# imatge-upc/rsis

Hardware: AMD Instinct MI355X
Metric: training images/sec at 256x256, T=10, batch=32 per GPU (higher is better)
Workload: dtype f32

## Files before the change

### rsis_amd/csrc/conv_wgrad_tiled.hip

```cpp
#include "common.h"
#include <stdlib.h>

typedef __attribute__((address_space(3))) void* lds_vp_t;

struct WgradTiledArgs {
  const float* dy;
  const float* x;
  float* dw;
  int B, Cs, H, W, Cout;
  int ldo, n_off, interleave_hid;
  int n_co_tiles, n_n_tiles, n_sp_tiles, tiles_per_split;
};

#define RSIS_OOB 0x7FFFFFF0u

template <int BM, int BN, int WGM, int WGN, int KS, int TW, int KSP = 1, int RAG = 0>
__device__ __forceinline__ void wgrad_tiled_body(const WgradTiledArgs& p, const int bx, const int by) {
#if __HIP_DEVICE_COMPILE__
  constexpr int TM = BM / WGM / 32, TN = BN / WGN / 32;
  constexpr int KK = KS * KS, HALO = KS / 2;
  constexpr int TP = KS == 1 ? 32 : 64;
  constexpr int TH = TP / TW;
  constexpr int NG = TP / 4;
  constexpr int GPR = TW / 4;
  constexpr int PW = TW + 2 * HALO, PH = TH + 2 * HALO, IMS = PW * PH;
  constexpr int CI_P = KS == 1 ? BN : (BN + KK - 2) / KK + 1;
  constexpr int AS = BM * TP;
  constexpr int XS = KS == 1 ? BN * TP : (CI_P * IMS + 255) / 256 * 256;
  constexpr int NA = BM * NG / 256;
  constexpr int NB4 = KS == 1 ? BN * NG / 256 : 0;
  constexpr int NB1 = KS == 1 ? 0 : XS / 256;
  static_assert(WGM * WGN * KSP == 4 && (BM * NG) % 256 == 0 && (KS == 3 || (BN * NG) % 256 == 0) && (NG / 2) % KSP == 0, "config");

  __shared__ __attribute__((aligned(16))) float lds[2 * (AS + XS)];
  float* const As0 = lds;
  float* const Xs0 = lds + 2 * AS;

  const int tid = threadIdx.x, lane = tid & 63, l31 = lane & 31, hi = lane >> 5;
  const int wave = __builtin_amdgcn_readfirstlane(tid >> 6);
  const int wk = wave / (WGM * WGN), wm = (wave % (WGM * WGN)) / WGN, wn = wave % WGN;
  const int H = p.H, W = p.W, HW = H * W, Cs = p.Cs, Cout = p.Cout;
  const int co_t = bx % p.n_co_tiles, n_t = bx / p.n_co_tiles;
  const int co0 = co_t * BM, n0 = n_t * BN;
  const int ci0 = n0 / KK;
  const int Nn = Cs * KK;
  const int tiles_x = RAG ? (W + TW - 1) / TW : W / TW, tiles_y = RAG ? (H + TH - 1) / TH : H / TH;
  const int rx = W - (tiles_x - 1) * TW, ry = H - (tiles_y - 1) * TH;
  const int t_begin = by * p.tiles_per_split;
  const int t_end = min(t_begin + p.tiles_per_split, p.n_sp_tiles);
  if (t_begin >= t_end) return;

  unsigned voa[NA];
#pragma unroll
  for (int i = 0; i < NA; ++i) {
    const int idx = tid + i * 256;
    const int row = idx / NG, sl = idx % NG;
    const int G = (sl & ~7) | ((sl & 7) ^ (row & 7));
    const int y = G / GPR, x4 = G % GPR;
    voa[i] = co0 + row < Cout ? ((unsigned)((co0 + row) * HW + y * W + x4 * 4) * 4u) | (RAG == 2 && x4 * 4 >= rx ? 1u : 0u) | (RAG == 2 && y >= ry ? 2u : 0u) : RSIS_OOB;
  }
  unsigned voa1[RAG == 1 ? 4 * NA : 1];
  unsigned vob1r[RAG == 1 && NB4 ? 4 * NB4 : 1];
  if constexpr (RAG == 1) {
#pragma unroll
    for (int k = 0; k < 4 * NA; ++k) {
      const int P = k * 256 + tid, idx = P >> 2, e = P & 3;
      const int row = idx / NG, sl = idx % NG;
      const int G = (sl & ~7) | ((sl & 7) ^ (row & 7));
      const int y = G / GPR, x = (G % GPR) * 4 + e;
      voa1[k] = co0 + row < Cout ? ((unsigned)((co0 + row) * HW + y * W + x) * 4u) | (x >= rx ? 1u : 0u) | (y >= ry ? 2u : 0u) : RSIS_OOB;
    }
    if constexpr (KS == 1) {
#pragma unroll
      for (int k = 0; k < 4 * NB4; ++k) {
        const int P = k * 256 + tid, idx = P >> 2, e = P & 3;
        const int row = idx / NG, sl = idx % NG;
        const int G = (sl & ~7) | ((sl & 7) ^ (row & 7));
        const int y = G / GPR, x = (G % GPR) * 4 + e;
        vob1r[k] = n0 + row < Cs ? ((unsigned)((n0 + row) * HW + y * W + x) * 4u) | (x >= rx ? 1u : 0u) | (y >= ry ? 2u : 0u) : RSIS_OOB;
      }
    }
  }
  unsigned vob4[NB4 ? NB4 : 1];
  unsigned vob1[NB1 ? NB1 : 1];
  unsigned cls1[NB1 ? NB1 : 1];
  if constexpr (KS == 1) {
#pragma unroll
    for (int i = 0; i < NB4; ++i) {
      const int idx = tid + i * 256;
      const int row = idx / NG, sl = idx % NG;
      const int G = (sl & ~7) | ((sl & 7) ^ (row & 7));
      const int y = G / GPR, x4 = G % GPR;
      vob4[i] = n0 + row < Cs ? ((unsigned)((n0 + row) * HW + y * W + x4 * 4) * 4u) | (RAG == 2 && x4 * 4 >= rx ? 1u : 0u) | (RAG == 2 && y >= ry ? 2u : 0u) : RSIS_OOB;
    }
  } else {
#pragma unroll
    for (int i = 0; i < NB1; ++i) {
      const int e = tid + i * 256;
      const int cl = e / IMS, rem = e - cl * IMS;
      const int py = rem / PW, pxx = rem - py * PW;
      const bool ok = cl < CI_P && ci0 + cl < Cs;
      vob1[i] = ok ? (unsigned)(cl * HW + py * W + pxx) * 4u : RSIS_OOB;
      cls1[i] = (py == 0 ? 1u : 0u) | (py - 1 >= ry ? 2u : 0u) | (pxx == 0 ? 4u : 0u) | (pxx - 1 >= rx ? 8u : 0u);
    }
  }

  int sg[NG / 2 / KSP];
  int bo[NG / 2 / KSP];
#pragma unroll
  for (int gg = 0; gg < NG / 2 / KSP; ++gg) {
    const int g = gg * KSP + (KSP == 1 ? 0 : wk);
    sg[gg] = ((2 * g + hi) ^ (l31 & 7)) * 4;
    bo[gg] = KS == 1 ? 0 : (g / (TW / 8)) * PW + (g % (TW / 8)) * 8;
  }
  const int arow = (wm * TM * 32 + l31) * TP;
  int xb[TN];
#pragma unroll
  for (int j = 0; j < TN; ++j) {
    const int nl = wn * TN * 32 + j * 32 + l31;
    if constexpr (KS == 1) {
      xb[j] = nl * TP;
    } else {
      const int n = n0 + nl;
      const int cl = n / KK - ci0, rs = n - (n / KK) * KK;
      xb[j] = cl * IMS + (rs / KS) * PW + (rs % KS) + 4 * hi;
    }
  }

  f32x16 acc[TM][TN];
#pragma unroll
  for (int i = 0; i < TM; ++i)
#pragma unroll
    for (int j = 0; j < TN; ++j)
#pragma unroll
      for (int r = 0; r < 16; ++r) acc[i][j][r] = 0.f;

  int tb = t_begin / (tiles_x * tiles_y);
  int trem = t_begin - tb * (tiles_x * tiles_y);
  int ty = trem / tiles_x, tx = trem - ty * tiles_x;

#define WG_ISSUE(BUF)                                                                                          \
  {                                                                                                            \
    const int y0 = ty * TH, x0 = tx * TW;                                                                      \
    const float* ab = p.dy + ((size_t)tb * Cout * HW + y0 * W + x0);                                           \
    const __amdgpu_buffer_rsrc_t ra_ = __builtin_amdgcn_make_buffer_rsrc((void*)ab, 0, 0x7FFFFFF0, 0x00020000); \
    const unsigned lastm = (tx == tiles_x - 1 ? 1u : 0u) | (ty == tiles_y - 1 ? 2u : 0u);                      \
    if constexpr (RAG == 1) {                                                                                  \
      float* As = As0 + (BUF) * AS + wave * 64;                                                                \
      _Pragma("unroll") for (int k = 0; k < 4 * NA; ++k)                                                       \
        __builtin_amdgcn_raw_ptr_buffer_load_lds(ra_, (lds_vp_t)(As + k * 256), 4, (voa1[k] & lastm) ? RSIS_OOB : (voa1[k] & ~3u), 0, 0, 0); \
    } else {                                                                                                   \
      float* As = As0 + (BUF) * AS + wave * 256;                                                               \
      _Pragma("unroll") for (int i = 0; i < NA; ++i)                                                           \
        __builtin_amdgcn_raw_ptr_buffer_load_lds(ra_, (lds_vp_t)(As + i * 1024), 16,                           \
                                                 RAG == 2 ? ((voa[i] & lastm) ? RSIS_OOB : (voa[i] & ~3u)) : voa[i], 0, 0, 0); \
    }                                                                                                          \
    if constexpr (KS == 1) {                                                                                   \
      const float* bb = p.x + ((size_t)tb * Cs * HW + y0 * W + x0);                                            \
      const __amdgpu_buffer_rsrc_t rb_ = __builtin_amdgcn_make_buffer_rsrc((void*)bb, 0, 0x7FFFFFF0, 0x00020000); \
      if constexpr (RAG == 1) {                                                                                \
        float* Xs = Xs0 + (BUF) * XS + wave * 64;                                                              \
        _Pragma("unroll") for (int k = 0; k < 4 * NB4; ++k)                                                    \
          __builtin_amdgcn_raw_ptr_buffer_load_lds(rb_, (lds_vp_t)(Xs + k * 256), 4, (vob1r[k] & lastm) ? RSIS_OOB : (vob1r[k] & ~3u), 0, 0, 0); \
      } else {                                                                                                 \
        float* Xs = Xs0 + (BUF) * XS + wave * 256;                                                             \
        _Pragma("unroll") for (int i = 0; i < NB4; ++i)                                                        \
          __builtin_amdgcn_raw_ptr_buffer_load_lds(rb_, (lds_vp_t)(Xs + i * 1024), 16,                         \
                                                   RAG == 2 ? ((vob4[i] & lastm) ? RSIS_OOB : (vob4[i] & ~3u)) : vob4[i], 0, 0, 0); \
      }                                                                                                        \
    } else {                                                                                                   \
      const float* bb = p.x + (((size_t)tb * Cs + ci0) * HW + (y0 - 1) * W + (x0 - 1));                        \
      const __amdgpu_buffer_rsrc_t rb_ = __builtin_amdgcn_make_buffer_rsrc((void*)bb, 0, 0x7FFFFFF0, 0x00020000); \
      const unsigned edge = (y0 == 0 ? 1u : 0u) | (ty == tiles_y - 1 ? 2u : 0u) | (x0 == 0 ? 4u : 0u) | (tx == tiles_x - 1 ? 8u : 0u); \
      float* Xs = Xs0 + (BUF) * XS + wave * 64;                                                                \
      _Pragma("unroll") for (int i = 0; i < NB1; ++i) {                                                        \
        const unsigned vo = (cls1[i] & edge) ? RSIS_OOB : vob1[i];                                             \
        __builtin_amdgcn_raw_ptr_buffer_load_lds(rb_, (lds_vp_t)(Xs + i * 256), 4, vo, 0, 0, 0);               \
      }                                                                                                        \
    }                                                                                                          \
    if (++tx == tiles_x) { tx = 0; if (++ty == tiles_y) { ty = 0; ++tb; } }                                    \
  }
#define WG_LAND() __builtin_amdgcn_s_waitcnt(0x0F70);

  WG_ISSUE(0)
  WG_LAND()
  __syncthreads();
  const int ntl = t_end - t_begin;
  for (int t = 0; t < ntl; ++t) {
    const int cur = t & 1;
    if (t + 1 < ntl) WG_ISSUE(cur ^ 1)
    {
      const float* As = As0 + cur * AS + arow;
      const float* Xs = Xs0 + cur * XS;
#pragma unroll
      for (int g = 0; g < NG / 2 / KSP; ++g) {
        f32x4 a4[TM];
#pragma unroll
        for (int i = 0; i < TM; ++i) a4[i] = *reinterpret_cast<const f32x4*>(As + i * 32 * TP + sg[g]);
        if constexpr (KS == 1) {
          f32x4 b4[TN];
#pragma unroll
          for (int j = 0; j < TN; ++j) b4[j] = *reinterpret_cast<const f32x4*>(Xs + xb[j] + sg[g]);
#pragma unroll
          for (int e = 0; e < 4; ++e)
#pragma unroll
            for (int i = 0; i < TM; ++i)
#pragma unroll
              for (int j = 0; j < TN; ++j) acc[i][j] = __builtin_amdgcn_mfma_f32_32x32x2f32(a4[i][e], b4[j][e], acc[i][j], 0, 0, 0);
        } else {
#pragma unroll
          for (int e = 0; e < 4; ++e) {
            float b[TN];
#pragma unroll
            for (int j = 0; j < TN; ++j) b[j] = Xs[xb[j] + (KSP == 1 ? (g / (TW / 8)) * PW + (g % (TW / 8)) * 8 : bo[g]) + e];
#pragma unroll
            for (int i = 0; i < TM; ++i)
#pragma unroll
              for (int j = 0; j < TN; ++j) acc[i][j] = __builtin_amdgcn_mfma_f32_32x32x2f32(a4[i][e], b[j], acc[i][j], 0, 0, 0);
          }
        }
      }
    }
    WG_LAND()
    __syncthreads();
  }
#undef WG_ISSUE
#undef WG_LAND

  const __amdgpu_buffer_rsrc_t rdw = __builtin_amdgcn_make_buffer_rsrc((void*)p.dw, 0, (unsigned)((size_t)Cout * p.ldo * 4), 0x00020000);
  const int ihid = p.interleave_hid;
  const unsigned ldb = (unsigned)p.ldo * 4u;
#pragma unroll
  for (int j = 0; j < TN; ++j) {
    const int n = n0 + wn * TN * 32 + j * 32 + l31;
    if (n >= Nn) continue;
#pragma unroll
    for (int i = 0; i < TM; ++i) {
      const int row0 = co0 + wm * TM * 32 + i * 32 + 4 * hi;
      const int rows_left = Cout - row0;
      const unsigned vo = (unsigned)((ihid > 0 ? row0 >> 2 : row0) * p.ldo + p.n_off + n) * 4u;
#pragma unroll
      for (int r = 0; r < 16; ++r) {
        const int k = (r & 3) + 8 * (r >> 2);
        const unsigned ro = (unsigned)(ihid > 0 ? (r & 3) * ihid + 2 * (r >> 2) : k) * ldb;
        __builtin_amdgcn_raw_ptr_buffer_atomic_fadd_f32(acc[i][j][r], rdw, k < rows_left ? vo + ro : 0x7FFFFFF0u, 0, 0);
      }
    }
  }
#endif
}

template <int BM, int BN, int WGM, int WGN, int KS, int TW, int KSP = 1>
__global__ __launch_bounds__(256) void conv_wgrad_tiled_kernel(const WgradTiledArgs p) {
  wgrad_tiled_body<BM, BN, WGM, WGN, KS, TW, KSP>(p, blockIdx.x, blockIdx.y);
}

#define RSIS_WG_MAXJ 48
struct WgradTiledGroup {
  int n;
  int begin[RSIS_WG_MAXJ + 1];
  WgradTiledArgs job[RSIS_WG_MAXJ];
};
static_assert(sizeof(WgradTiledGroup) <= 4000, "kernel arguments are limited to 4 KB");

template <int BM, int BN, int WGM, int WGN, int KS, int TW, int KSP = 1, int RAG = 0>
__global__ __launch_bounds__(256) void conv_wgrad_tiled_group_kernel(const WgradTiledGroup g) {
  const int b = blockIdx.x;
  int lo = 0, hi = g.n - 1;
  while (lo < hi) {
    const int mid = (lo + hi + 1) >> 1;
    if (g.begin[mid] <= b) lo = mid; else hi = mid - 1;
  }
  const WgradTiledArgs& p = g.job[lo];
  const int local = b - g.begin[lo];
  const int ntile = p.n_co_tiles * p.n_n_tiles;
  wgrad_tiled_body<BM, BN, WGM, WGN, KS, TW, KSP, RAG>(p, local % ntile, local / ntile);
}

template <int BM, int BN, int WGM, int WGN, int KS, int TW, int KSP = 1>
static int launch_tiled_cfg(WgradTiledArgs& a, hipStream_t st) {
  constexpr int TH = (KS == 1 ? 32 : 64) / TW;
  a.n_co_tiles = rsis_cdiv(a.Cout, BM);
  a.n_n_tiles = rsis_cdiv((long)a.Cs * KS * KS, BN);
  a.n_sp_tiles = a.B * (a.H / TH) * (a.W / TW);
  const int ntile = a.n_co_tiles * a.n_n_tiles;
  const int slots = KS == 1 ? (BM * BN >= 128 * 128 ? 256 : 512) : 256 * (BM * BN >= 128 * 128 ? 2 : 3);
  int nsplit = ntile >= slots ? 1 : slots / ntile;
  if (nsplit > a.n_sp_tiles / 2) nsplit = a.n_sp_tiles / 2;
  if (nsplit < 1 || rsis_deterministic()) nsplit = 1;
  a.tiles_per_split = rsis_cdiv(a.n_sp_tiles, nsplit);
  nsplit = rsis_cdiv(a.n_sp_tiles, a.tiles_per_split);
  hipLaunchKernelGGL((conv_wgrad_tiled_kernel<BM, BN, WGM, WGN, KS, TW, KSP>), dim3(ntile, nsplit), dim3(256), 0, st, a);
  return rsis_check_launch();
}

template <int KS, int TW>
static int launch_tiled_tw(WgradTiledArgs& a, hipStream_t st) {
  const int nmod = (a.Cs * KS * KS) % 128;
  const bool narrow = nmod != 0 && nmod <= 64;
  if (rsis_deterministic() && a.Cout <= 32) return launch_tiled_cfg<32, 128, 1, 4, KS, TW>(a, st);
  if (KS == 1 && a.Cout > 32) return launch_tiled_cfg<64, 64, 2, 2, KS, TW>(a, st);
  if (a.Cout <= 32) return narrow ? launch_tiled_cfg<32, 64, 1, 2, KS, TW, 2>(a, st) : launch_tiled_cfg<32, 128, 1, 4, KS, TW>(a, st);
  if (a.Cout <= 64) return narrow ? launch_tiled_cfg<64, 64, 2, 2, KS, TW>(a, st) : launch_tiled_cfg<64, 128, 2, 2, KS, TW>(a, st);
  return narrow ? launch_tiled_cfg<128, 64, 2, 2, KS, TW>(a, st) : launch_tiled_cfg<128, 128, 2, 2, KS, TW>(a, st);
}

static int tiled_tw(int H, int W, int ks) {
  const int tp = ks == 1 ? 32 : 64;
  for (int tw = ks == 1 ? 32 : 16; tw >= 8; tw >>= 1)
    if (W % tw == 0 && H % (tp / tw) == 0) return tw;
  return 0;
}
static int tiled_tw_ragged(int W, int ks) {
  const int wide = ks == 1 ? 32 : 16;
  return W > 16 ? wide : (W > 8 ? 16 : 8);
}

static int tiled_cfg_code(const WgradTiledArgs& a, int ks) {
  const int nmod = (a.Cs * ks * ks) % 128;
  const bool narrow = nmod != 0 && nmod <= 64;
  if (ks == 1 && a.Cout > 32) return 2;
  if (a.Cout <= 32) return narrow && !rsis_deterministic() ? 0 : 1;
  if (a.Cout <= 64) return narrow ? 2 : 3;
  return narrow ? 4 : 5;
}

template <int BM, int BN, int WGM, int WGN, int KS, int TW, int KSP = 1, int RAG = 0>
static int launch_group_cfg(WgradTiledArgs* jobs, int n, hipStream_t st) {
  constexpr int TH = (KS == 1 ? 32 : 64) / TW;
  long total_iters = 0;
  for (int j = 0; j < n; ++j) {
    WgradTiledArgs& a = jobs[j];
    a.n_co_tiles = rsis_cdiv(a.Cout, BM);
    a.n_n_tiles = rsis_cdiv((long)a.Cs * KS * KS, BN);
    a.n_sp_tiles = RAG ? a.B * rsis_cdiv(a.H, TH) * rsis_cdiv(a.W, TW) : a.B * (a.H / TH) * (a.W / TW);
    total_iters += (long)a.n_co_tiles * a.n_n_tiles * a.n_sp_tiles;
  }
  static const int env_tb = getenv("RSIS_WG_GROUP_BLOCKS") ? atoi(getenv("RSIS_WG_GROUP_BLOCKS")) : 0;
  const long target_blocks = env_tb > 0 ? env_tb : 2048;
  long L = (total_iters + target_blocks - 1) / target_blocks;
  if (L < 2) L = 2;
  if (rsis_deterministic()) L = 1L << 40;
  for (int j0 = 0; j0 < n; j0 += RSIS_WG_MAXJ) {
    WgradTiledGroup g;
    g.n = n - j0 < RSIS_WG_MAXJ ? n - j0 : RSIS_WG_MAXJ;
    int blocks = 0;
    for (int j = 0; j < g.n; ++j) {
      WgradTiledArgs a = jobs[j0 + j];
      int nsplit = rsis_cdiv(a.n_sp_tiles, L);
      if (nsplit < 1) nsplit = 1;
      a.tiles_per_split = rsis_cdiv(a.n_sp_tiles, nsplit);
      nsplit = rsis_cdiv(a.n_sp_tiles, a.tiles_per_split);
      g.begin[j] = blocks;
      g.job[j] = a;
      blocks += a.n_co_tiles * a.n_n_tiles * nsplit;
    }
    g.begin[g.n] = blocks;
    hipLaunchKernelGGL((conv_wgrad_tiled_group_kernel<BM, BN, WGM, WGN, KS, TW, KSP, RAG>), dim3(blocks), dim3(256), 0, st, g);
    if (rsis_check_launch() != RSIS_OK) return RSIS_ERR_LAUNCH;
  }
  return RSIS_OK;
}

template <int KS, int TW, int RAG = 0>
static int launch_group_tw(int code, WgradTiledArgs* jobs, int n, hipStream_t st) {
  switch (code) {
    case 0: return launch_group_cfg<32, 64, 1, 2, KS, TW, 2, RAG>(jobs, n, st);
    case 1: return launch_group_cfg<32, 128, 1, 4, KS, TW, 1, RAG>(jobs, n, st);
    case 2: return launch_group_cfg<64, 64, 2, 2, KS, TW, 1, RAG>(jobs, n, st);
    case 3: return launch_group_cfg<64, 128, 2, 2, KS, TW, 1, RAG>(jobs, n, st);
    case 4: return launch_group_cfg<128, 64, 2, 2, KS, TW, 1, RAG>(jobs, n, st);
    default: return launch_group_cfg<128, 128, 2, 2, KS, TW, 1, RAG>(jobs, n, st);
  }
}

int rsis_launch_conv_wgrad_tiled_group(const WgradArgs* w, int n, int ks, hipStream_t st) {
  if (n < 1) return RSIS_OK;
  WgradTiledArgs* all = (WgradTiledArgs*)malloc(sizeof(WgradTiledArgs) * n * 2);
  int* key = (int*)malloc(sizeof(int) * n);
  if (!all || !key) { free(all); free(key); return RSIS_ERR_LAUNCH; }
  WgradTiledArgs* bucket = all + n;
  for (int j = 0; j < n; ++j) {
    WgradTiledArgs a = {};
    a.dy = w[j].dy; a.x = w[j].x; a.dw = w[j].dw; a.B = w[j].B; a.Cs = w[j].Cs; a.H = w[j].H; a.W = w[j].W; a.Cout = w[j].Cout;
    a.ldo = w[j].ldo; a.n_off = w[j].n_off; a.interleave_hid = w[j].interleave_hid;
    all[j] = a;
    const int twa = tiled_tw(a.H, a.W, ks);
    if (twa) key[j] = twa * 8 + tiled_cfg_code(a, ks);
    else {
      if (ks == 1 && (a.H * a.W) % 4 == 0) { all[j].W = a.W = a.H * a.W; all[j].H = a.H = 1; }
      key[j] = (a.W % 4 == 0 ? 2048 : 1024) + tiled_tw_ragged(a.W, ks) * 8 + tiled_cfg_code(a, ks);
    }
  }
  int rc = RSIS_OK;
  for (int j = 0; j < n && rc == RSIS_OK; ++j) {
    if (key[j] < 0) continue;
    const int k = key[j];
    int m = 0;
    for (int i = j; i < n; ++i)
      if (key[i] == k) { bucket[m++] = all[i]; key[i] = -1; }
    const int rag = k >> 10;
    const int tw = (k & 1023) / 8, code = k % 8;
    if (rag == 1) {
      if (ks == 1) rc = tw == 32 ? launch_group_tw<1, 32, 1>(code, bucket, m, st) : (tw == 16 ? launch_group_tw<1, 16, 1>(code, bucket, m, st) : launch_group_tw<1, 8, 1>(code, bucket, m, st));
      else rc = tw == 16 ? launch_group_tw<3, 16, 1>(code, bucket, m, st) : launch_group_tw<3, 8, 1>(code, bucket, m, st);
    } else if (rag == 2) {
      if (ks == 1) rc = tw == 32 ? launch_group_tw<1, 32, 2>(code, bucket, m, st) : (tw == 16 ? launch_group_tw<1, 16, 2>(code, bucket, m, st) : launch_group_tw<1, 8, 2>(code, bucket, m, st));
      else rc = tw == 16 ? launch_group_tw<3, 16, 2>(code, bucket, m, st) : launch_group_tw<3, 8, 2>(code, bucket, m, st);
    } else if (ks == 1) rc = tw == 32 ? launch_group_tw<1, 32>(code, bucket, m, st) : (tw == 16 ? launch_group_tw<1, 16>(code, bucket, m, st) : launch_group_tw<1, 8>(code, bucket, m, st));
    else rc = tw == 16 ? launch_group_tw<3, 16>(code, bucket, m, st) : launch_group_tw<3, 8>(code, bucket, m, st);
  }
  free(all); free(key);
  return rc;
}

bool rsis_wgrad_tiled_supported(const WgradArgs& w, int ks) {
  if (!(ks == 1 || ks == 3) || w.stride != 1 || w.pad != ks / 2 || w.H != w.Ho || w.W != w.Wo) return false;
  static const bool ragged_on = !(getenv("RSIS_WGRAD_RAGGED") && getenv("RSIS_WGRAD_RAGGED")[0] == '0');
  if (tiled_tw(w.H, w.W, ks) == 0 && !ragged_on) return false;
  const long img = (long)w.H * w.W * 4;
  return (long)w.Cout * img < (1L << 30) && (long)w.Cs * img < (1L << 30);
}

int rsis_launch_conv_wgrad_tiled(const WgradArgs& w, int ks, hipStream_t st) {
  WgradTiledArgs a = {};
  a.dy = w.dy; a.x = w.x; a.dw = w.dw; a.B = w.B; a.Cs = w.Cs; a.H = w.H; a.W = w.W; a.Cout = w.Cout;
  a.ldo = w.ldo; a.n_off = w.n_off; a.interleave_hid = w.interleave_hid;
  const int tw = tiled_tw(w.H, w.W, ks);
  if (tw == 0) return rsis_launch_conv_wgrad_tiled_group(&w, 1, ks, st);
  if (ks == 1) {
    if (tw == 32) return launch_tiled_tw<1, 32>(a, st);
    if (tw == 16) return launch_tiled_tw<1, 16>(a, st);
    return launch_tiled_tw<1, 8>(a, st);
  }
  if (tw == 16) return launch_tiled_tw<3, 16>(a, st);
  return launch_tiled_tw<3, 8>(a, st);
}
```

Before: 905.7.

## Emulate fp32 wgrad MFMA with three-limb bf16 split products

Adds a limb path to the tiled weight-gradient kernel. Each fp32 operand is split into three truncated bf16 limbs, and six cross products are accumulated with 32x32x16 bf16 MFMA in place of the fp32 32x32x2 MFMA. The path is enabled by default only for selected kernel-size, tile-width and config codes, and an environment variable can override it. The aim is to use the much higher bf16 matrix throughput while keeping accuracy close to fp32, at the cost of extra split and pack ALU work per LDS load and slightly lower precision from dropping the low-order limb products.

```diff
diff --git a/rsis_amd/csrc/conv_wgrad_tiled.hip b/rsis_amd/csrc/conv_wgrad_tiled.hip
--- a/rsis_amd/csrc/conv_wgrad_tiled.hip
+++ b/rsis_amd/csrc/conv_wgrad_tiled.hip
@@ -1,7 +1,30 @@
 #include "common.h"
+#include "limb_split.h"
 #include <stdlib.h>
+#include <string.h>
 
 typedef __attribute__((address_space(3))) void* lds_vp_t;
+typedef __bf16 wg_bf16x8 __attribute__((ext_vector_type(8)));
+typedef unsigned wg_u32x4 __attribute__((ext_vector_type(4)));
+
+#define WG_LIMB_PRODUCTS 6
+[[maybe_unused]] __device__ constexpr int wg_limb_pa[9] = {2, 1, 0, 1, 0, 0, 2, 1, 2};
+[[maybe_unused]] __device__ constexpr int wg_limb_pb[9] = {0, 1, 2, 0, 1, 0, 1, 2, 2};
+
+__device__ __forceinline__ void wg_limb_pack8(const float (&v)[8], wg_bf16x8 (&out)[3]) {
+  wg_u32x4 q[3];
+#pragma unroll
+  for (int m = 0; m < 4; ++m) {
+    float lo[3], hi[3];
+    rsis_limb_split3(v[2 * m], lo[0], lo[1], lo[2]);
+    rsis_limb_split3(v[2 * m + 1], hi[0], hi[1], hi[2]);
+    q[0][m] = __builtin_amdgcn_perm(__float_as_uint(v[2 * m + 1]), __float_as_uint(v[2 * m]), 0x07060302u);
+    q[1][m] = __builtin_amdgcn_perm(__float_as_uint(hi[1]), __float_as_uint(lo[1]), 0x07060302u);
+    q[2][m] = __builtin_amdgcn_perm(__float_as_uint(hi[2]), __float_as_uint(lo[2]), 0x07060302u);
+  }
+#pragma unroll
+  for (int l = 0; l < 3; ++l) out[l] = __builtin_bit_cast(wg_bf16x8, q[l]);
+}
 
 struct WgradTiledArgs {
   const float* dy;
@@ -14,7 +37,7 @@
 
 #define RSIS_OOB 0x7FFFFFF0u
 
-template <int BM, int BN, int WGM, int WGN, int KS, int TW, int KSP = 1, int RAG = 0>
+template <int BM, int BN, int WGM, int WGN, int KS, int TW, int KSP = 1, int RAG = 0, int LIMB = 0>
 __device__ __forceinline__ void wgrad_tiled_body(const WgradTiledArgs& p, const int bx, const int by) {
 #if __HIP_DEVICE_COMPILE__
   constexpr int TM = BM / WGM / 32, TN = BN / WGN / 32;
@@ -30,7 +53,7 @@
   constexpr int NA = BM * NG / 256;
   constexpr int NB4 = KS == 1 ? BN * NG / 256 : 0;
   constexpr int NB1 = KS == 1 ? 0 : XS / 256;
-  static_assert(WGM * WGN * KSP == 4 && (BM * NG) % 256 == 0 && (KS == 3 || (BN * NG) % 256 == 0) && (NG / 2) % KSP == 0, "config");
+  static_assert(WGM * WGN * KSP == 4 && (BM * NG) % 256 == 0 && (KS == 3 || (BN * NG) % 256 == 0) && (NG / 2) % KSP == 0 && (NG / 2 / KSP) % 2 == 0, "config");
 
   __shared__ __attribute__((aligned(16))) float lds[2 * (AS + XS)];
   float* const As0 = lds;
@@ -192,6 +215,43 @@
     {
       const float* As = As0 + cur * AS + arow;
       const float* Xs = Xs0 + cur * XS;
+      if constexpr (LIMB) {
+#pragma unroll
+        for (int g = 0; g < NG / 2 / KSP; g += 2) {
+          wg_bf16x8 al[TM][3], bl[TN][3];
+#pragma unroll
+          for (int i = 0; i < TM; ++i) {
+            const f32x4 a0 = *reinterpret_cast<const f32x4*>(As + i * 32 * TP + sg[g]);
+            const f32x4 a1 = *reinterpret_cast<const f32x4*>(As + i * 32 * TP + sg[g + 1]);
+            const float v[8] = {a0[0], a0[1], a0[2], a0[3], a1[0], a1[1], a1[2], a1[3]};
+            wg_limb_pack8(v, al[i]);
+          }
+#pragma unroll
+          for (int j = 0; j < TN; ++j) {
+            float v[8];
+            if constexpr (KS == 1) {
+              const f32x4 b0 = *reinterpret_cast<const f32x4*>(Xs + xb[j] + sg[g]);
+              const f32x4 b1 = *reinterpret_cast<const f32x4*>(Xs + xb[j] + sg[g + 1]);
+#pragma unroll
+              for (int e = 0; e < 4; ++e) { v[e] = b0[e]; v[4 + e] = b1[e]; }
+            } else {
+#pragma unroll
+              for (int u = 0; u < 2; ++u)
+#pragma unroll
+                for (int e = 0; e < 4; ++e)
+                  v[4 * u + e] = Xs[xb[j] + (KSP == 1 ? ((g + u) / (TW / 8)) * PW + ((g + u) % (TW / 8)) * 8 : bo[g + u]) + e];
+            }
+            wg_limb_pack8(v, bl[j]);
+          }
+#pragma unroll
+          for (int q = 0; q < WG_LIMB_PRODUCTS; ++q)
+#pragma unroll
+            for (int i = 0; i < TM; ++i)
+#pragma unroll
+              for (int j = 0; j < TN; ++j)
+                acc[i][j] = __builtin_amdgcn_mfma_f32_32x32x16_bf16(al[i][wg_limb_pa[q]], bl[j][wg_limb_pb[q]], acc[i][j], 0, 0, 0);
+        }
+      } else
 #pragma unroll
       for (int g = 0; g < NG / 2 / KSP; ++g) {
         f32x4 a4[TM];
@@ -250,9 +310,9 @@
 #endif
 }
 
-template <int BM, int BN, int WGM, int WGN, int KS, int TW, int KSP = 1>
+template <int BM, int BN, int WGM, int WGN, int KS, int TW, int KSP = 1, int LIMB = 0>
 __global__ __launch_bounds__(256) void conv_wgrad_tiled_kernel(const WgradTiledArgs p) {
-  wgrad_tiled_body<BM, BN, WGM, WGN, KS, TW, KSP>(p, blockIdx.x, blockIdx.y);
+  wgrad_tiled_body<BM, BN, WGM, WGN, KS, TW, KSP, 0, LIMB>(p, blockIdx.x, blockIdx.y);
 }
 
 #define RSIS_WG_MAXJ 48
@@ -263,7 +323,7 @@
 };
 static_assert(sizeof(WgradTiledGroup) <= 4000, "kernel arguments are limited to 4 KB");
 
-template <int BM, int BN, int WGM, int WGN, int KS, int TW, int KSP = 1, int RAG = 0>
+template <int BM, int BN, int WGM, int WGN, int KS, int TW, int KSP = 1, int RAG = 0, int LIMB = 0>
 __global__ __launch_bounds__(256) void conv_wgrad_tiled_group_kernel(const WgradTiledGroup g) {
   const int b = blockIdx.x;
   int lo = 0, hi = g.n - 1;
@@ -274,10 +334,25 @@
   const WgradTiledArgs& p = g.job[lo];
   const int local = b - g.begin[lo];
   const int ntile = p.n_co_tiles * p.n_n_tiles;
-  wgrad_tiled_body<BM, BN, WGM, WGN, KS, TW, KSP, RAG>(p, local % ntile, local / ntile);
-}
-
-template <int BM, int BN, int WGM, int WGN, int KS, int TW, int KSP = 1>
+  wgrad_tiled_body<BM, BN, WGM, WGN, KS, TW, KSP, RAG, LIMB>(p, local % ntile, local / ntile);
+}
+
+static unsigned wg_limb_mask(int ks, int tw) {
+  if (ks == 3) return tw == 16 ? 0x3Fu : (tw == 8 ? 1u << 5 : 0u);
+  return tw == 16 || tw == 8 ? 1u << 2 : 0u;
+}
+static bool wg_use_limbs(int ks, int tw, int code, int rag) {
+  static const int mode = [] {
+    const char* e = getenv("RSIS_WGRAD_LIMBS");
+    if (!e || !e[0]) return 0;
+    if (e[0] == '0') return 1;
+    return strcmp(e, "all") == 0 ? 2 : 0;
+  }();
+  if (mode) return mode == 2;
+  return rag == 0 && ((wg_limb_mask(ks, tw) >> code) & 1u);
+}
+
+template <int BM, int BN, int WGM, int WGN, int KS, int TW, int KSP = 1, int LIMB = 0>
 static int launch_tiled_cfg(WgradTiledArgs& a, hipStream_t st) {
   constexpr int TH = (KS == 1 ? 32 : 64) / TW;
   a.n_co_tiles = rsis_cdiv(a.Cout, BM);
@@ -290,19 +365,28 @@
   if (nsplit < 1 || rsis_deterministic()) nsplit = 1;
   a.tiles_per_split = rsis_cdiv(a.n_sp_tiles, nsplit);
   nsplit = rsis_cdiv(a.n_sp_tiles, a.tiles_per_split);
-  hipLaunchKernelGGL((conv_wgrad_tiled_kernel<BM, BN, WGM, WGN, KS, TW, KSP>), dim3(ntile, nsplit), dim3(256), 0, st, a);
+  hipLaunchKernelGGL((conv_wgrad_tiled_kernel<BM, BN, WGM, WGN, KS, TW, KSP, LIMB>), dim3(ntile, nsplit), dim3(256), 0, st, a);
   return rsis_check_launch();
 }
+
+template <int KS, int TW, int LIMB>
+static int launch_tiled_code(int code, WgradTiledArgs& a, hipStream_t st) {
+  switch (code) {
+    case 0: return launch_tiled_cfg<32, 64, 1, 2, KS, TW, 2, LIMB>(a, st);
+    case 1: return launch_tiled_cfg<32, 128, 1, 4, KS, TW, 1, LIMB>(a, st);
+    case 2: return launch_tiled_cfg<64, 64, 2, 2, KS, TW, 1, LIMB>(a, st);
+    case 3: return launch_tiled_cfg<64, 128, 2, 2, KS, TW, 1, LIMB>(a, st);
+    case 4: return launch_tiled_cfg<128, 64, 2, 2, KS, TW, 1, LIMB>(a, st);
+    default: return launch_tiled_cfg<128, 128, 2, 2, KS, TW, 1, LIMB>(a, st);
+  }
+}
+
+static int tiled_cfg_code(const WgradTiledArgs& a, int ks);
 
 template <int KS, int TW>
 static int launch_tiled_tw(WgradTiledArgs& a, hipStream_t st) {
-  const int nmod = (a.Cs * KS * KS) % 128;
-  const bool narrow = nmod != 0 && nmod <= 64;
-  if (rsis_deterministic() && a.Cout <= 32) return launch_tiled_cfg<32, 128, 1, 4, KS, TW>(a, st);
-  if (KS == 1 && a.Cout > 32) return launch_tiled_cfg<64, 64, 2, 2, KS, TW>(a, st);
-  if (a.Cout <= 32) return narrow ? launch_tiled_cfg<32, 64, 1, 2, KS, TW, 2>(a, st) : launch_tiled_cfg<32, 128, 1, 4, KS, TW>(a, st);
-  if (a.Cout <= 64) return narrow ? launch_tiled_cfg<64, 64, 2, 2, KS, TW>(a, st) : launch_tiled_cfg<64, 128, 2, 2, KS, TW>(a, st);
-  return narrow ? launch_tiled_cfg<128, 64, 2, 2, KS, TW>(a, st) : launch_tiled_cfg<128, 128, 2, 2, KS, TW>(a, st);
+  const int code = tiled_cfg_code(a, KS);
+  return wg_use_limbs(KS, TW, code, 0) ? launch_tiled_code<KS, TW, 1>(code, a, st) : launch_tiled_code<KS, TW, 0>(code, a, st);
 }
 
 static int tiled_tw(int H, int W, int ks) {
@@ -325,7 +409,7 @@
   return narrow ? 4 : 5;
 }
 
-template <int BM, int BN, int WGM, int WGN, int KS, int TW, int KSP = 1, int RAG = 0>
+template <int BM, int BN, int WGM, int WGN, int KS, int TW, int KSP = 1, int RAG = 0, int LIMB = 0>
 static int launch_group_cfg(WgradTiledArgs* jobs, int n, hipStream_t st) {
   constexpr int TH = (KS == 1 ? 32 : 64) / TW;
   long total_iters = 0;
@@ -356,22 +440,27 @@
       blocks += a.n_co_tiles * a.n_n_tiles * nsplit;
     }
     g.begin[g.n] = blocks;
-    hipLaunchKernelGGL((conv_wgrad_tiled_group_kernel<BM, BN, WGM, WGN, KS, TW, KSP, RAG>), dim3(blocks), dim3(256), 0, st, g);
+    hipLaunchKernelGGL((conv_wgrad_tiled_group_kernel<BM, BN, WGM, WGN, KS, TW, KSP, RAG, LIMB>), dim3(blocks), dim3(256), 0, st, g);
     if (rsis_check_launch() != RSIS_OK) return RSIS_ERR_LAUNCH;
   }
   return RSIS_OK;
+}
+
+template <int KS, int TW, int RAG, int LIMB>
+static int launch_group_code(int code, WgradTiledArgs* jobs, int n, hipStream_t st) {
+  switch (code) {
+    case 0: return launch_group_cfg<32, 64, 1, 2, KS, TW, 2, RAG, LIMB>(jobs, n, st);
+    case 1: return launch_group_cfg<32, 128, 1, 4, KS, TW, 1, RAG, LIMB>(jobs, n, st);
+    case 2: return launch_group_cfg<64, 64, 2, 2, KS, TW, 1, RAG, LIMB>(jobs, n, st);
+    case 3: return launch_group_cfg<64, 128, 2, 2, KS, TW, 1, RAG, LIMB>(jobs, n, st);
+    case 4: return launch_group_cfg<128, 64, 2, 2, KS, TW, 1, RAG, LIMB>(jobs, n, st);
+    default: return launch_group_cfg<128, 128, 2, 2, KS, TW, 1, RAG, LIMB>(jobs, n, st);
+  }
 }
 
 template <int KS, int TW, int RAG = 0>
 static int launch_group_tw(int code, WgradTiledArgs* jobs, int n, hipStream_t st) {
-  switch (code) {
-    case 0: return launch_group_cfg<32, 64, 1, 2, KS, TW, 2, RAG>(jobs, n, st);
-    case 1: return launch_group_cfg<32, 128, 1, 4, KS, TW, 1, RAG>(jobs, n, st);
-    case 2: return launch_group_cfg<64, 64, 2, 2, KS, TW, 1, RAG>(jobs, n, st);
-    case 3: return launch_group_cfg<64, 128, 2, 2, KS, TW, 1, RAG>(jobs, n, st);
-    case 4: return launch_group_cfg<128, 64, 2, 2, KS, TW, 1, RAG>(jobs, n, st);
-    default: return launch_group_cfg<128, 128, 2, 2, KS, TW, 1, RAG>(jobs, n, st);
-  }
+  return wg_use_limbs(KS, TW, code, RAG) ? launch_group_code<KS, TW, RAG, 1>(code, jobs, n, st) : launch_group_code<KS, TW, RAG, 0>(code, jobs, n, st);
 }
 
 int rsis_launch_conv_wgrad_tiled_group(const WgradArgs* w, int n, int ks, hipStream_t st) {
diff --git a/rsis_amd/csrc/limb_split.h b/rsis_amd/csrc/limb_split.h
--- /dev/null
+++ b/rsis_amd/csrc/limb_split.h
@@ -0,0 +1,23 @@
+#pragma once
+
+#if defined(__HIPCC__) || defined(__CUDACC__)
+#define RSIS_LIMB_HD __host__ __device__
+#else
+#define RSIS_LIMB_HD
+#endif
+
+RSIS_LIMB_HD inline float rsis_limb_hi16(const float v) {
+  unsigned u;
+  __builtin_memcpy(&u, &v, 4);
+  u &= 0xFFFF0000u;
+  float r;
+  __builtin_memcpy(&r, &u, 4);
+  return r;
+}
+
+RSIS_LIMB_HD inline void rsis_limb_split3(const float v, float& l0, float& l1, float& l2) {
+  l0 = rsis_limb_hi16(v);
+  const float r1 = v - l0;
+  l1 = rsis_limb_hi16(r1);
+  l2 = r1 - l1;
+}
```

Measured after the change: 944.6 (median of 6 runs). 1.04x the previous value.
